# ctlab/metafast

Hardware: AMD Instinct MI355X
Metric: k-mers/s counted+graphed at k=31, 150 bp reads (higher is better)
Workload: dtype u64

## Files before the change

### metafast_amd/csrc/mf_skm.hip

```cpp
#include "mf_common.h"
#include "mf_count_dev.h"
#include <algorithm>
#include <memory>
#include <vector>
#include "mf_skm_scan.h"
#include "mf_skm_scatter.h"
#include "mf_skm_split.h"
#include "mf_skm_count.h"

template <typename KF> static int skm_set_lds(KF kern, size_t bytes) {
    MF_HIP(hipFuncSetAttribute(reinterpret_cast<const void *>(kern), hipFuncAttributeMaxDynamicSharedMemorySize, (int)bytes));
    return MF_OK;
}

#define SKM_PILOT_CH 8192
__global__ __launch_bounds__(256) void k_skm_pilot(const skm_rec *__restrict__ recs, const uint64_t *__restrict__ pstart, const uint32_t *__restrict__ plen,
                                                   const uint32_t *__restrict__ regions, int shift, uint32_t nsel, uint32_t *__restrict__ cnt,
                                                   uint32_t *__restrict__ occ, const uint64_t *__restrict__ ostart, uint32_t *__restrict__ cur,
                                                   skm_rec *__restrict__ out) {
    extern __shared__ uint32_t sh[];
    const uint32_t rg = blockIdx.y, d1 = regions[rg];
    const uint64_t start = pstart[d1];
    const uint32_t len = plen[d1];
    const uint32_t j0 = blockIdx.x * (uint32_t)SKM_PILOT_CH;
    if (j0 >= len) return;
    const uint32_t j1 = min(len, j0 + (uint32_t)SKM_PILOT_CH);
    const bool hist = ostart == nullptr;
    if (hist) { for (uint32_t i = threadIdx.x; i < 2u * nsel; i += blockDim.x) sh[i] = 0; __syncthreads(); }
    for (uint32_t j = j0 + threadIdx.x; j < j1; j += blockDim.x) {
        const skm_rec v = recs[start + j];
        if (!skm_rec_valid(v)) continue;
        const uint32_t d = skm_rec_digits(v) >> shift;
        if (d >= nsel) continue;
        if (hist) { atomicAdd(&sh[d], 1u); atomicAdd(&sh[nsel + d], skm_rec_n(v)); }
        else { const uint32_t at = atomicAdd(&cur[rg * nsel + d], 1u); out[ostart[rg * nsel + d] + at] = v; }
    }
    if (hist) {
        __syncthreads();
        for (uint32_t i = threadIdx.x; i < nsel; i += blockDim.x) {
            if (sh[i]) { atomicAdd(&cnt[rg * nsel + i], sh[i]); atomicAdd(&occ[rg * nsel + i], sh[nsel + i]); }
        }
    }
}
__global__ void k_skm_pilot_dir(const uint32_t *__restrict__ cnt, uint32_t n, uint32_t *__restrict__ plen) {
    const uint32_t i = blockIdx.x * blockDim.x + threadIdx.x;
    if (i < n) plen[i] = (cnt[i] + 3u) & ~3u;
}
template <int K>
static int skm_pilot(mf_ctx *ctx, const skm_rec *bufA, const uint64_t *pstart, const uint32_t *plen, uint32_t dlo, uint32_t dhi, uint64_t n_occ, int nd1,
                     int bits_planned, int kthr, double *rho, double *kept, double *rec_per_occ) {
    hipStream_t st = ctx->stream;
    *rho = -1.0; *kept = -1.0; *rec_per_occ = 0.0;
    if (dhi <= dlo) return MF_OK;
    const uint32_t R = std::min<uint32_t>(8u, dhi - dlo);
    const int pb = std::min((int)SKM_DIGIT_BITS, bits_planned + 3);
    const double per_unit = (double)n_occ / (double)nd1 / (double)(1u << pb);
    uint32_t nsel = (uint32_t)std::min<double>((double)(1u << pb), std::max(1.0, std::ceil(2.5e6 / (per_unit * R))));
    if (nsel > 2048u) nsel = 2048u;
    const uint32_t nb = R * nsel;
    std::vector<uint32_t> h_reg(R);
    for (uint32_t i = 0; i < R; i++) h_reg[i] = dlo + (uint32_t)(((uint64_t)(2 * i + 1) * (dhi - dlo)) / (2 * R));
    std::vector<uint32_t> h_len(nd1);
    mf_buf<uint32_t> reg, cnt, occ, cur, uplen, dcount; mf_buf<uint64_t> ostart, toff; mf_buf<unsigned long long> ps;
    MF_TRY(reg.alloc(ctx, R)); MF_TRY(cnt.alloc(ctx, (size_t)3 * nb)); MF_TRY(uplen.alloc(ctx, nb)); MF_TRY(dcount.alloc(ctx, nb));
    MF_TRY(ostart.alloc(ctx, (size_t)nb + 1)); MF_TRY(toff.alloc(ctx, (size_t)nb + 1)); MF_TRY(ps.alloc(ctx, 24));
    uint32_t *const d_cnt = cnt.p, *const d_occ = cnt.p + nb, *const d_cur = cnt.p + 2 * (size_t)nb;
    MF_HIP(hipMemcpyAsync(reg.p, h_reg.data(), (size_t)R * 4, hipMemcpyHostToDevice, st));
    MF_HIP(hipMemsetAsync(cnt.p, 0, (size_t)3 * nb * 4, st));
    MF_HIP(hipMemsetAsync(ps.p, 0, 24 * 8, st));
    const uint64_t mean_len = std::max<uint64_t>(1, n_occ / (uint64_t)nd1 / 4);
    const unsigned gx = (unsigned)std::min<uint64_t>(65535, (4 * mean_len + SKM_PILOT_CH - 1) / SKM_PILOT_CH + 1);
    const int shift = SKM_DIGIT_BITS - pb;
    mf_ktimer tm(ctx, "k_skm_pilot");
    k_skm_pilot<<<dim3(gx, R), 256, (size_t)2 * nsel * 4, st>>>(bufA, pstart, plen, reg.p, shift, nsel, d_cnt, d_occ, nullptr, nullptr, nullptr);
    k_skm_pilot_dir<<<(nb + 255) / 256, 256, 0, st>>>(d_cnt, nb, uplen.p);
    MF_TRY(mf_scan<1>(ctx, uplen.p, ostart.p, nb, (uint64_t *)&ps.p[0]));
    MF_TRY(mf_scan<1>(ctx, d_occ, toff.p, nb, (uint64_t *)&ps.p[1]));
    unsigned long long tot[2] = {0, 0};
    MF_HIP(hipMemcpyAsync(tot, ps.p, 16, hipMemcpyDeviceToHost, st));
    MF_HIP(hipStreamSynchronize(st));
    if (!tot[0] || !tot[1]) return MF_OK;
    mf_buf<skm_rec> pr; mf_buf<uint64_t> tkeys; mf_buf<uint16_t> tcnt;
    if (pr.alloc(ctx, tot[0] + 4) != MF_OK || tkeys.alloc(ctx, tot[1]) != MF_OK || tcnt.alloc(ctx, tot[1]) != MF_OK) return MF_OK;
    MF_HIP(hipMemsetAsync(pr.p, 0xFF, (tot[0] + 4) * sizeof(skm_rec), st));
    k_skm_pilot<<<dim3(gx, R), 256, 0, st>>>(bufA, pstart, plen, reg.p, shift, nsel, nullptr, nullptr, ostart.p, d_cur, pr.p);
    {
        const unsigned grid = (unsigned)std::min<uint64_t>(nb, (uint64_t)ctx->n_cu * C2_WG_PER_CU);
        k_skm_count<K><<<grid, SKM_CT, C2_LDS, st>>>(pr.p, ostart.p, uplen.p, nb, toff.p, tkeys.p, tcnt.p, dcount.p, (unsigned int *)&ps.p[2], 0u, (uint64_t)0, kthr,
                                                         &ps.p[3], (unsigned int *)&ps.p[4], nullptr, &ps.p[8], (uint64_t)tot[1], (uint32_t)ctx->opt_skm_dedupe, nullptr);
    }
    MF_TRY(mf_scan<1>(ctx, dcount.p, ostart.p, nb, (uint64_t *)&ps.p[5]));
    unsigned long long res[4] = {0, 0, 0, 0};
    MF_HIP(hipMemcpyAsync(res, &ps.p[2], 32, hipMemcpyDeviceToHost, st));
    MF_HIP(hipStreamSynchronize(st));
    MF_HIP(hipGetLastError());
    const bool over = (res[0] & 0xFFFFFFFFull) != 0;
    *rho = over ? 1.0 : (double)res[1] / (double)tot[1];
    if (!over) *kept = (double)res[3] / (double)tot[1];
    *rec_per_occ = (double)tot[0] / (double)tot[1];
    if (ctx->opt_verbose)
        fprintf(stderr, "[mf] skm pilot: %u would-be units of %u regions (2^%d per region): %llu records, %llu occurrences, %llu distinct k-mers = %.4f per occurrence (%llu kept), %llu unit(s) redone\n",
                nb, R, pb, tot[0], tot[1], res[1], *rho, res[3], res[2] & 0xFFFFFFFFull);
    return MF_OK;
}

struct skm_snap_slice {
    std::vector<uint64_t> rec;
    std::vector<uint64_t> pstart, l1_pstart; std::vector<uint32_t> plen, pocc, l1_plen;
    std::vector<int> lv;
    uint64_t cap = 0, wpb = 0, n_valid = 0; uint32_t dlo = 0, dhi = 0; int G = 0, one_pass = 0, repeated = 0, fast = 0;
};
struct mf_skm_snap { std::vector<skm_snap_slice> slices; };
#define MF_SKM_SNAPPED 3
struct skm_acc {
    mf_skm_snap *snap = nullptr;
    mf_buf<uint64_t> dk; mf_buf<uint16_t> dc; uint64_t dused = 0, dcap = 0;
    mf_buf<uint64_t> doff;
    mf_buf<unsigned long long> dhist, c2p;
    unsigned long long n_records = 0, cap_l1 = 0;
    uint32_t np_total = 0;
    int split_bits = 1;
    int table_bits = 0;
};
#define MF_SKM_NOMEM 2
struct skm_shared {
    uint32_t lo = 0, hi = 0;
    bool ready = false;
    mf_buf<skm_rec> buf; mf_buf<uint64_t> pstart; mf_buf<uint32_t> plen, pocc;
    std::vector<uint64_t> h_pstart;
    unsigned long long cap = 0;
    void clear() { buf.reset(); pstart.reset(); plen.reset(); pocc.reset(); h_pstart.clear(); ready = false; cap = 0; }
};
struct skm_reads { const uint8_t *bases; uint64_t n_bases; const uint32_t *vmask; uint64_t n_words; };
struct skm_job { skm_reads in; uint64_t n_occ; unsigned long long *scal; int kthr; };
struct skm_l1 { skm_reads in; uint64_t wpb; int bits1, G; uint32_t lo, hi; size_t fast_lds; };
struct skm_slice_state {
    std::vector<int> &lv; int total_bits;
    uint32_t dlo, dhi;
    skm_l1 l1;
    uint32_t np; mf_buf<uint64_t> pstart; mf_buf<uint32_t> plen, pocc;
    mf_buf<skm_rec> bufA; unsigned long long cap = 0;
    uint64_t rebase = 0;
    int snap_one_pass = 0, snap_repeated = 0;
};
#define SKM_STEP(call) do { const int rc__ = (call); if (rc__ != MF_OK) return rc__; } while (0)

static size_t skm_fast_lds(const mf_ctx *ctx, int nd1) {
    const size_t fast_lds = ((skm_stage_bytes(nd1) + 15) & ~(size_t)15) + (size_t)16 * SKM_FAST_WAVE_BYTES;
    return fast_lds > (size_t)160 * 1024 || ctx->opt_scatter_fast == 0 ? 0 : fast_lds;
}
template <int K, bool DYN>
static int skm_scatter(mf_ctx *ctx, const skm_l1 &L, const uint64_t *blockstart, skm_rec *out, const skm_dyn &Dy) {
    hipStream_t st = ctx->stream;
    mf_ktimer t(ctx, "k_skm_scatter");
    if (L.fast_lds) {
        MF_TRY(skm_set_lds(k_skm_scatter<K, DYN, true>, L.fast_lds));
        k_skm_scatter<K, DYN, true><<<L.G, 1024, L.fast_lds, st>>>(L.in.bases, L.in.n_bases, L.in.vmask, L.in.n_words, L.wpb, L.bits1, blockstart, L.G, out, Dy, L.lo, L.hi);
    } else {
        const size_t lds = skm_stage_bytes(1 << L.bits1);
        MF_TRY(skm_set_lds(k_skm_scatter<K, DYN, false>, lds));
        k_skm_scatter<K, DYN, false><<<L.G, 1024, lds, st>>>(L.in.bases, L.in.n_bases, L.in.vmask, L.in.n_words, L.wpb, L.bits1, blockstart, L.G, out, Dy, L.lo, L.hi);
    }
    return MF_OK;
}
static unsigned long long skm_final_cap(const std::vector<int> &lv, uint64_t n_occ, unsigned long long c1, bool headroom) {
    const int nd1 = 1 << lv[0];
    if (headroom) return c1 + n_occ / 128 + (unsigned long long)nd1 * SKM_LINE * (1ull << MF_MAX_DIGIT_BITS);
    if (lv.size() < 3) return c1;
    unsigned long long c = c1, p = (unsigned long long)nd1;
    for (size_t li = 1; li < lv.size(); li++) { c += p * SKM_LINE * (1ull << lv[li]); p <<= lv[li]; }
    return c;
}

template <int K>
static int skm_level1(mf_ctx *ctx, const skm_job &J, skm_slice_state &T, bool own, bool headroom) {
    hipStream_t st = ctx->stream;
    unsigned long long *const scal = J.scal;
    const skm_l1 &L = T.l1;
    const int bits1 = L.bits1, nd1 = 1 << bits1, G = L.G;
    const uint32_t np = T.np;
    const bool l1_only = T.lv.size() == 1;
    auto final_cap = [&](unsigned long long c1) { return skm_final_cap(T.lv, J.n_occ, c1, headroom); };
    unsigned long long &cap = T.cap;
    bool dyn = !l1_only && (ctx->opt_skm_dyn == 2 || (ctx->opt_skm_dyn == 1 && L.in.n_words >= (1ull << 24)));
    for (int attempt = dyn ? 0 : 1; attempt < 2; attempt++) {
        const bool D = attempt == 0;
        const int stride = D ? (ctx->opt_skm_dyn == 2 ? 3 : 16) : 1;
        mf_buf<uint32_t> blockhist; MF_TRY(blockhist.alloc(ctx, (size_t)nd1 * G));
        mf_buf<uint32_t> blockocc; if (l1_only) MF_TRY(blockocc.alloc(ctx, (size_t)nd1 * G));
        {
            mf_ktimer t(ctx, D ? "k_skm_hist_sample" : "k_skm_hist");
            k_skm_hist<K><<<G, 1024, (size_t)nd1 * 8, st>>>(L.in.bases, L.in.n_bases, L.in.vmask, L.in.n_words, L.wpb, bits1, blockhist.p, blockocc.p, G, stride, L.lo, L.hi);
        }
        MF_DBG(ctx, "k_skm_hist");
        if (D) {
            mf_buf<uint32_t> rsize; MF_TRY(rsize.alloc(ctx, np));
            mf_buf<uint64_t> rstart; MF_TRY(rstart.alloc(ctx, (size_t)np + 1));
            mf_buf<unsigned long long> gcur; MF_TRY(gcur.alloc(ctx, np));
            k_skm_region_sizes<<<(nd1 + 255) / 256, 256, 0, st>>>(blockhist.p, G, nd1, (uint32_t)stride, rsize.p, L.lo, L.hi);
            MF_TRY(mf_scan<1>(ctx, rsize.p, rstart.p, np, (uint64_t *)&scal[1]));
            MF_HIP(hipMemcpyAsync(gcur.p, rstart.p, (size_t)np * 8, hipMemcpyDeviceToDevice, st));
            MF_HIP(hipMemsetAsync(&scal[5], 0, 8, st));
            MF_HIP(hipMemcpyAsync(&cap, &scal[1], 8, hipMemcpyDeviceToHost, st));
            MF_HIP(hipStreamSynchronize(st));
            if (T.bufA.alloc(ctx, std::max<unsigned long long>(cap + (uint64_t)G * SKM_CH, own ? final_cap(cap) : 0ull)) != MF_OK) return MF_SKM_NOMEM;
            skm_dyn Dy; Dy.gcur = gcur.p; Dy.rend = rstart.p + 1; Dy.overflow = (unsigned int *)&scal[5]; Dy.dump = cap; Dy.save = nullptr;
            MF_TRY((skm_scatter<K, true>(ctx, L, nullptr, T.bufA.p, Dy)));
            MF_DBG(ctx, "k_skm_scatter");
            k_skm_dir_dyn<<<(nd1 + 255) / 256, 256, 0, st>>>(rstart.p, gcur.p, nd1, T.pstart.p, T.plen.p);
            unsigned long long ovf = 0;
            MF_HIP(hipMemcpyAsync(&ovf, &scal[5], 8, hipMemcpyDeviceToHost, st));
            MF_HIP(hipStreamSynchronize(st));
            if (!ovf) { T.snap_one_pass = 1; break; }
            T.snap_repeated = 1;
            if (ctx->opt_verbose) fprintf(stderr, "[mf] skm: a sampled digit region was too small, level 1 again with exact ranges\n");
            T.bufA.reset();
            continue;
        }
        mf_buf<uint64_t> blockstart; MF_TRY(blockstart.alloc(ctx, (size_t)nd1 * G + 1));
        MF_TRY(mf_scan<SKM_LINE>(ctx, blockhist.p, blockstart.p, (uint64_t)nd1 * G, (uint64_t *)&scal[1]));
        MF_HIP(hipMemcpyAsync(&cap, &scal[1], 8, hipMemcpyDeviceToHost, st));
        MF_HIP(hipStreamSynchronize(st));
        if (T.bufA.alloc(ctx, own ? final_cap(cap) : cap) != MF_OK) return MF_SKM_NOMEM;
        MF_TRY((skm_scatter<K, false>(ctx, L, blockstart.p, T.bufA.p, skm_dyn())));
        MF_DBG(ctx, "k_skm_scatter");
        k_skm_dir<<<(nd1 + 255) / 256, 256, 0, st>>>(blockstart.p, blockocc.p, G, nd1, T.pstart.p, T.plen.p, T.pocc.p);
    }
    return MF_OK;
}

template <int K>
static int skm_share_level1(mf_ctx *ctx, skm_slice_state &T, skm_shared *SH, uint64_t n_occ) {
    hipStream_t st = ctx->stream;
    const int nd1 = 1 << T.l1.bits1;
    if (!SH->ready) {
        SH->buf.swap(T.bufA); SH->pstart.swap(T.pstart); SH->plen.swap(T.plen); SH->pocc.swap(T.pocc);
        SH->cap = T.cap;
        SH->h_pstart.resize(nd1);
        MF_HIP(hipMemcpyAsync(SH->h_pstart.data(), SH->pstart.p, (size_t)nd1 * 8, hipMemcpyDeviceToHost, st));
        MF_HIP(hipStreamSynchronize(st));
        SH->ready = true;
        if (T.l1.lo == 0 && T.l1.hi == (uint32_t)nd1 && n_occ) { ctx->last_l1_per_occ = (double)SH->cap / (double)n_occ; ctx->last_l1_k = K; }
    }
    T.bufA.borrow(ctx, SH->buf.p, SH->buf.n);
    MF_TRY(T.pstart.alloc(ctx, T.np)); MF_TRY(T.plen.alloc(ctx, T.np)); MF_TRY(T.pocc.alloc(ctx, T.np));
    MF_HIP(hipMemcpyAsync(T.pstart.p, SH->pstart.p, (size_t)nd1 * 8, hipMemcpyDeviceToDevice, st));
    MF_HIP(hipMemcpyAsync(T.plen.p, SH->plen.p, (size_t)nd1 * 4, hipMemcpyDeviceToDevice, st));
    T.rebase = SH->h_pstart[T.dlo];
    T.cap = (T.dhi < (uint32_t)nd1 ? SH->h_pstart[T.dhi] : SH->cap) - T.rebase;
    return MF_OK;
}

template <int K>
static int skm_replan_from_pilot(mf_ctx *ctx, const skm_job &J, skm_slice_state &T, skm_acc &A, bool *split_from_pilot) {
    const uint64_t n_occ = J.n_occ;
    const int kthr = J.kthr, bits1 = T.l1.bits1, nd1 = 1 << bits1;
    std::vector<int> &lv = T.lv;
    int &total_bits = T.total_bits;
    double rho = -1.0, kept = -1.0, rpo = 0.0;
    MF_TRY(skm_pilot<K>(ctx, T.bufA.p, T.pstart.p, T.plen.p, T.dlo, T.dhi, n_occ, nd1, total_bits - bits1, kthr, &rho, &kept, &rpo));
    ctx->last_pilot_rho = rho; ctx->n_pilots++;
    if (rho > 0.0) {
        double want_units = (double)n_occ * rho / (double)std::max<int64_t>(64, ctx->opt_skm_unit_distinct);
        const int64_t unit_records = ctx->opt_skm_unit_records > 0 ? ctx->opt_skm_unit_records : (K >= 25 ? 2000 : 4000) * SKM_CT / 512;
        if (ctx->opt_skm_dedupe) want_units = std::max(want_units, (double)n_occ * rpo / (double)unit_records);
        int Bc = 0; while (Bc < 30 && (double)(1ull << Bc) < want_units) Bc++;
        const int r = std::max(1, std::min(Bc - bits1, std::min((int)SKM_DIGIT_BITS, 30 - bits1)));
        if (ctx->opt_verbose) fprintf(stderr, "[mf] skm pilot: %.4f distinct k-mers per occurrence -> %d bits after level 1 (planned from the occurrences alone: %d)\n", rho, r, total_bits - bits1);
        lv.resize(1);
        if (r <= MF_MAX_DIGIT_BITS) lv.push_back(r); else { lv.push_back((r + 1) / 2); lv.push_back(r / 2); }
        total_bits = 0; for (int b : lv) total_bits += b;
        if (kthr >= 0 && kept >= 0.0 && !A.doff.p) {
            const double per_unit = (double)n_occ * kept / (double)(1ull << total_bits);
            int sb = 0; while (sb < 4 && per_unit / (double)(1 << sb) > (double)ctx->opt_part_good) sb++;
            A.split_bits = sb; *split_from_pilot = true;
            if (ctx->opt_verbose) fprintf(stderr, "[mf] skm pilot: %.4f k-mers per occurrence survive the cut: %.0f per counting unit -> %d table partition(s) per unit\n", kept, per_unit, 1 << sb);
        }
    }
    return MF_OK;
}

static int skm_plan_table(mf_ctx *ctx, int total_bits, bool split_from_pilot, skm_acc &A) {
    if (!split_from_pilot) A.split_bits = A.table_bits > 0 ? std::max(0, std::min(4, A.table_bits - total_bits)) : 1;
    if (total_bits + A.split_bits > 30) A.split_bits = 30 - total_bits;
    A.np_total = (uint32_t)(1ull << (total_bits + A.split_bits));
    MF_TRY(A.doff.alloc(ctx, (size_t)A.np_total + 1));
    return MF_OK;
}

static int skm_restrict_to_slice(mf_ctx *ctx, skm_slice_state &T) {
    hipStream_t st = ctx->stream;
    const uint32_t dlo = T.dlo, np = T.dhi - T.dlo;
    T.np = np;
    mf_buf<uint64_t> ps; MF_TRY(ps.alloc(ctx, np)); mf_buf<uint32_t> pl, po; MF_TRY(pl.alloc(ctx, np)); MF_TRY(po.alloc(ctx, np));
    MF_HIP(hipMemcpyAsync(ps.p, T.pstart.p + dlo, (size_t)np * 8, hipMemcpyDeviceToDevice, st));
    MF_HIP(hipMemcpyAsync(pl.p, T.plen.p + dlo, (size_t)np * 4, hipMemcpyDeviceToDevice, st));
    MF_HIP(hipMemcpyAsync(po.p, T.pocc.p + dlo, (size_t)np * 4, hipMemcpyDeviceToDevice, st));
    T.pstart.swap(ps); T.plen.swap(pl); T.pocc.swap(po);
    return MF_OK;
}

static int skm_snapshot_level1(mf_ctx *ctx, const skm_slice_state &T, skm_snap_slice &snap) {
    hipStream_t st = ctx->stream;
    const uint32_t np = T.np;
    snap.l1_pstart.resize(np); snap.l1_plen.resize(np);
    MF_HIP(hipMemcpyAsync(snap.l1_pstart.data(), T.pstart.p, (size_t)np * 8, hipMemcpyDeviceToHost, st));
    MF_HIP(hipMemcpyAsync(snap.l1_plen.data(), T.plen.p, (size_t)np * 4, hipMemcpyDeviceToHost, st));
    MF_HIP(hipStreamSynchronize(st));
// ... 783 lines not shown
```

### metafast_amd/csrc/mf_skm_scan.h

```cpp
#pragma once
#include "mf_common.h"
#include "mf_count_dev.h"

typedef ulonglong2 skm_rec;
typedef uint32_t skm_v4 __attribute__((ext_vector_type(4)));
#define SKM_LINE 4
#define SKM_QCAP 16
#define SKM_DIGIT_BITS 22
#define SKM_CT 512
#define SKM_NW (SKM_CT / 64)

__device__ __forceinline__ bool skm_rec_valid(const skm_rec &r) { return ((uint32_t)r.y & 63u) != 63u; }
__device__ __forceinline__ uint32_t skm_rec_n(const skm_rec &r) { return (uint32_t)r.y & 63u; }
__device__ __forceinline__ uint32_t skm_rec_digits(const skm_rec &r) { return (uint32_t)(r.y >> 6) & ((1u << SKM_DIGIT_BITS) - 1u); }

template <int K> struct skm_word {
    static constexpr int W = K - mf_skm_m(K) + 1;
    static constexpr int NM = 31 + W;
    static constexpr int RMAX = (MF_SKM_BASES - (K - 1)) < 20 ? (MF_SKM_BASES - (K - 1)) : 20;
    uint32_t D[4];
    uint32_t mh[32];
    uint32_t valid;
    uint32_t cut;
};

template <int K>
__device__ __forceinline__ void skm_cut_mask(skm_word<K> &S, uint32_t m) {
    uint32_t acc = 0;
#pragma unroll
    for (int j = 31; j >= 1; j--)
        asm("v_cmp_eq_u32 vcc, %1, %2\n\tv_addc_co_u32 %0, vcc, %0, %0, vcc" : "+v"(acc) : "v"(S.mh[j]), "v"(S.mh[j - 1]) : "vcc");
    const uint32_t same = acc << 1;
    S.cut = m & ~(same & (m << 1));
}

__device__ __forceinline__ uint32_t skm_rc16(uint32_t d) {
    const uint32_t r = __brev(~d);
    return ((r & 0xAAAAAAAAu) >> 1) | ((r & 0x55555555u) << 1);
}
template <int M>
__device__ __forceinline__ uint32_t skm_mmer_at(const uint32_t (&X)[4], int p) {
    const int q = p >> 4, o = p & 15;
    const uint32_t top = o ? __builtin_amdgcn_alignbit(X[q], q + 1 < 4 ? X[q + 1] : 0u, 32 - 2 * o) : X[q];
    return top >> (32 - 2 * M);
}

template <int K>
__device__ __forceinline__ void skm_scan_tail(skm_word<K> &S, uint32_t (&hs)[skm_word<K>::NM], uint32_t m) {
    constexpr int W = skm_word<K>::W, NM = skm_word<K>::NM;
    static_assert(W >= 3 && W <= 18, "window");
    auto min3 = [](uint32_t a, uint32_t b, uint32_t c) { const uint32_t m = a < b ? a : b; return m < c ? m : c; };
#pragma unroll
    for (int i = 0; i + 2 < NM; i++) hs[i] = min3(hs[i], hs[i + 1], hs[i + 2]);
    if (W >= 9) {
#pragma unroll
        for (int i = 0; i + 8 < NM; i++) hs[i] = min3(hs[i], hs[i + 3], hs[i + 6]);
#pragma unroll
        for (int j = 0; j < 32; j++) S.mh[j] = hs[j] < hs[j + W - 9] ? hs[j] : hs[j + W - 9];
    } else {
        constexpr int D = W - 3 < 3 ? W - 3 : 3;
#pragma unroll
        for (int j = 0; j < 32; j++) S.mh[j] = min3(hs[j], hs[j + D], hs[j + W - 3]);
    }
    skm_cut_mask<K>(S, m);
}

template <int K>
__device__ __forceinline__ void skm_scan_word(skm_word<K> &S, const uint8_t *__restrict__ bases, uint64_t n_bases, uint64_t w, uint32_t m) {
    constexpr int NM = skm_word<K>::NM, M = mf_skm_m(K);
    const uint64_t b0 = w * 32;
    const uint4 *p = reinterpret_cast<const uint4 *>(bases + (b0 < n_bases ? b0 : 0));
    const bool in1 = b0 + 16 < n_bases, in2 = b0 + 32 < n_bases, in3 = b0 + 48 < n_bases;
    const uint4 c0 = p[0], c1 = p[in1 ? 1 : 0], c2 = p[in2 ? 2 : 0], c3 = p[in3 ? 3 : 0];
    S.D[0] = b0 < n_bases ? mf_dec16(c0) : 0u; S.D[1] = in1 ? mf_dec16(c1) : 0u; S.D[2] = in2 ? mf_dec16(c2) : 0u; S.D[3] = in3 ? mf_dec16(c3) : 0u;
    S.valid = m;
    uint32_t hs[NM];
    const uint32_t R[4] = {skm_rc16(S.D[3]), skm_rc16(S.D[2]), skm_rc16(S.D[1]), skm_rc16(S.D[0])};
#pragma unroll
    for (int i = 0; i < NM; i++) {
        const uint32_t f = skm_mmer_at<M>(S.D, i), r = skm_mmer_at<M>(R, 64 - M - i);
        hs[i] = mf_mmer_hash(f < r ? f : r, M);
    }
    skm_scan_tail<K>(S, hs, m);
}
__device__ __forceinline__ uint32_t skm_from_next_lane(uint32_t v) {
    return (uint32_t)__builtin_amdgcn_update_dpp(0, (int)v, 0x130 , 0xF, 0xF, false);
}
__device__ __forceinline__ uint32_t skm_from_prev_lane(uint32_t v) {
    return (uint32_t)__builtin_amdgcn_update_dpp(0, (int)v, 0x138 , 0xF, 0xF, false);
}
template <int K>
__device__ __forceinline__ void skm_scan_word_halo(skm_word<K> &S, const uint8_t *__restrict__ bases, uint64_t n_bases, uint64_t w, uint32_t m) {
    constexpr int NM = skm_word<K>::NM, M = mf_skm_m(K);
    const uint64_t b0 = w * 32;
    const uint4 *p = reinterpret_cast<const uint4 *>(bases + (b0 < n_bases ? b0 : 0));
    const bool in1 = b0 + 16 < n_bases;
    const uint4 c0 = p[0], c1 = p[in1 ? 1 : 0];
    S.D[0] = b0 < n_bases ? mf_dec16(c0) : 0u; S.D[1] = in1 ? mf_dec16(c1) : 0u;
    S.D[2] = skm_from_next_lane(S.D[0]); S.D[3] = skm_from_next_lane(S.D[1]);
    S.valid = m;
    static_assert(64 - M - 31 >= 16, "reversed words");
    const uint32_t R3 = skm_rc16(S.D[0]);
    const uint32_t R[4] = {0u, skm_from_next_lane(R3), skm_rc16(S.D[1]), R3};
    uint32_t hs[34];
#pragma unroll
    for (int i = 0; i < 32; i++) {
        const uint32_t f = skm_mmer_at<M>(S.D, i), r = skm_mmer_at<M>(R, 64 - M - i);
        hs[i] = mf_mmer_hash(f < r ? f : r, M);
    }
    constexpr int W = skm_word<K>::W;
    static_assert(W >= 3 && W <= 18, "window");
    static_assert(NM <= 64, "halo");
    auto min3 = [](uint32_t a, uint32_t b, uint32_t c) { const uint32_t m = a < b ? a : b; return m < c ? m : c; };
    hs[32] = skm_from_next_lane(hs[0]); hs[33] = skm_from_next_lane(hs[1]);
    uint32_t a[38];
#pragma unroll
    for (int i = 0; i < 32; i++) a[i] = min3(hs[i], hs[i + 1], hs[i + 2]);
    if (W >= 9) {
        uint32_t b[32 + 9];
#pragma unroll
        for (int i = 32; i < 38; i++) a[i] = skm_from_next_lane(a[i - 32]);
#pragma unroll
        for (int i = 0; i < 32; i++) b[i] = min3(a[i], a[i + 3], a[i + 6]);
#pragma unroll
        for (int i = 32; i < 32 + W - 9; i++) b[i] = skm_from_next_lane(b[i - 32]);
#pragma unroll
        for (int j = 0; j < 32; j++) S.mh[j] = b[j] < b[j + W - 9] ? b[j] : b[j + W - 9];
    } else {
        constexpr int D = W - 3 < 3 ? W - 3 : 3;
#pragma unroll
        for (int i = 32; i < 32 + W - 3; i++) a[i] = skm_from_next_lane(a[i - 32]);
#pragma unroll
        for (int j = 0; j < 32; j++) S.mh[j] = min3(a[j], a[j + D], a[j + W - 3]);
    }
    skm_cut_mask<K>(S, m);
}

__device__ __forceinline__ uint32_t skm_sel(uint32_t a, uint32_t b, unsigned long long m) {
    uint32_t r;
    asm("v_cndmask_b32 %0, %1, %2, %3" : "=v"(r) : "v"(a), "v"(b), "s"(m));
    return r;
}
template <int K>
__device__ __forceinline__ uint32_t skm_mh_at(const skm_word<K> &S, uint32_t s) {
    uint32_t a[16], b[8], c[4], d[2];
    const unsigned long long s0 = __ballot((s & 1u) != 0), s1 = __ballot((s & 2u) != 0), s2 = __ballot((s & 4u) != 0),
                             s3 = __ballot((s & 8u) != 0), s4 = __ballot((s & 16u) != 0);
#pragma unroll
    for (int i = 0; i < 16; i++) a[i] = skm_sel(S.mh[2 * i], S.mh[2 * i + 1], s0);
#pragma unroll
    for (int i = 0; i < 8; i++) b[i] = skm_sel(a[2 * i], a[2 * i + 1], s1);
#pragma unroll
    for (int i = 0; i < 4; i++) c[i] = skm_sel(b[2 * i], b[2 * i + 1], s2);
#pragma unroll
    for (int i = 0; i < 2; i++) d[i] = skm_sel(c[2 * i], c[2 * i + 1], s3);
    return skm_sel(d[0], d[1], s4);
}

template <int K>
__device__ __forceinline__ void skm_next_run(const skm_word<K> &S, uint32_t &cut, uint32_t &s, uint32_t &len) {
    s = (uint32_t)__builtin_ctz(cut);
    cut &= cut - 1u;
    const uint32_t stop = (cut | ~S.valid) & ~((2u << s) - 1u);
    const uint32_t e = stop ? (uint32_t)__builtin_ctz(stop) : 32u;
    len = e - s;
    if (len > (uint32_t)skm_word<K>::RMAX) { len = (uint32_t)skm_word<K>::RMAX; cut |= 1u << (s + len); }
}

template <int K>
__device__ __forceinline__ skm_rec skm_make_rec(const uint32_t (&D)[4], uint32_t s, uint32_t len, uint32_t digits, uint32_t D4 = 0u) {
    const uint32_t o = (2u * s) & 31u;
    const unsigned long long q = __ballot(s >= 16u);
    const uint32_t E0 = skm_sel(D[0], D[1], q), E1 = skm_sel(D[1], D[2], q), E2 = skm_sel(D[2], D[3], q), E3 = skm_sel(D[3], D4, q), E4 = skm_sel(D4, 0u, q);
    uint32_t T0 = E0, T1 = E1, T2 = E2, T3 = E3;
    if (o) {
        T0 = __builtin_amdgcn_alignbit(E0, E1, 32u - o);
        T1 = __builtin_amdgcn_alignbit(E1, E2, 32u - o);
        T2 = __builtin_amdgcn_alignbit(E2, E3, 32u - o);
        T3 = __builtin_amdgcn_alignbit(E3, E4, 32u - o);
    }
    static_assert(K >= 17 && K <= 32, "the first dword is kept whole");
    const int kb = 2 * (int)(len + K - 1);
    const uint64_t m01 = (uint64_t)((int64_t)0x8000000000000000ull >> ((kb < 64 ? kb : 64) - 1));
    const uint64_t m23 = ~(~0ull >> (kb > 64 ? kb - 64 : 0));
    T1 &= (uint32_t)m01; T2 &= (uint32_t)(m23 >> 32); T3 &= (uint32_t)m23;
    skm_rec r;
    r.x = ((uint64_t)T0 << 32) | T1;
    r.y = ((uint64_t)T2 << 32) | (uint64_t)(T3 & 0xF0000000u) | ((uint64_t)digits << 6) | (uint64_t)len;
    return r;
}
__device__ __forceinline__ void skm_route(uint32_t mh, int bits1, uint32_t &d1, uint32_t &digits) {
    const uint32_t ph = mf_remix32(mh);
    d1 = bits1 ? ph >> (32 - bits1) : 0u;
    digits = (bits1 ? (ph << bits1) : ph) >> (32 - SKM_DIGIT_BITS);
}
```

### metafast_amd/csrc/mf_skm_scatter.h

```cpp
#pragma once
#include "mf_skm_scan.h"

template <int K>
__global__ __launch_bounds__(1024) void k_skm_hist(const uint8_t *__restrict__ bases, uint64_t n_bases, const uint32_t *__restrict__ vmask,
                                                   uint64_t n_words, uint64_t words_per_block, int bits1,
                                                   uint32_t *__restrict__ blockhist, uint32_t *__restrict__ blockocc, int G, int stride,
                                                   uint32_t dlo, uint32_t dhi) {
    extern __shared__ __attribute__((aligned(16))) unsigned char smem[];
    const int nd = 1 << bits1;
    uint32_t *hist = reinterpret_cast<uint32_t *>(smem), *occ = hist + nd;
    for (int i = threadIdx.x; i < 2 * nd; i += blockDim.x) hist[i] = 0;
    __syncthreads();
    const uint64_t wlo = (uint64_t)blockIdx.x * words_per_block;
    const uint64_t whi = wlo + words_per_block < n_words ? wlo + words_per_block : n_words;
    for (uint64_t wb = wlo; wb < whi; wb += (uint64_t)blockDim.x * (uint64_t)stride) {
        const uint64_t w = wb + threadIdx.x;
        const uint32_t m = w < whi ? vmask[w] : 0u;
        if (__ballot(m != 0u) == 0ull) continue;
        skm_word<K> S;
        skm_scan_word<K>(S, bases, n_bases, w < n_words ? w : 0, m);
        uint32_t cut = S.cut;
        while (__ballot(cut != 0u) != 0ull) {
            if (cut) {
                uint32_t s, len, d1, digits;
// ... 40 lines not shown
                 "s_mov_b64 exec, %5\n\tds_read_b32 %0, %9\n\t"
                 "s_mov_b64 exec, %6\n\tds_read_b32 %1, %10\n\t"
                 "s_mov_b64 exec, %7\n\tds_read_b32 %2, %11\n\t"
                 "s_mov_b64 exec, %8\n\tds_read_b32 %3, %12\n\t"
                 "s_mov_b64 exec, %4\n\ts_waitcnt lgkmcnt(0)"
                 : "=&v"(v[0]), "=&v"(v[1]), "=&v"(v[2]), "=&v"(v[3]), "=&s"(sv)
                 : "s"(m[0]), "s"(m[1]), "s"(m[2]), "s"(m[3]), "v"(a[0]), "v"(a[1]), "v"(a[2]), "v"(a[3])
                 : "memory");
}
__device__ __forceinline__ void skm_lds_add_rtn4_if(const unsigned long long (&m)[4], const uint32_t (&a)[4], uint32_t inc, uint32_t (&old)[4]) {
    unsigned long long sv;
    asm volatile("s_mov_b64 %4, exec\n\t"
                 "s_mov_b64 exec, %5\n\tds_add_rtn_u32 %0, %9, %13\n\t"
                 "s_mov_b64 exec, %6\n\tds_add_rtn_u32 %1, %10, %13\n\t"
                 "s_mov_b64 exec, %7\n\tds_add_rtn_u32 %2, %11, %13\n\t"
                 "s_mov_b64 exec, %8\n\tds_add_rtn_u32 %3, %12, %13\n\t"
                 "s_mov_b64 exec, %4\n\ts_waitcnt lgkmcnt(0)"
                 : "=&v"(old[0]), "=&v"(old[1]), "=&v"(old[2]), "=&v"(old[3]), "=&s"(sv)
                 : "s"(m[0]), "s"(m[1]), "s"(m[2]), "s"(m[3]), "v"(a[0]), "v"(a[1]), "v"(a[2]), "v"(a[3]), "v"(inc)
                 : "memory");
}
__device__ __forceinline__ void skm_lds_write4_add_rtn4_if(const unsigned long long (&m)[4], const uint32_t (&wa)[4], const skm_v4 (&wv)[4],
                                                           const uint32_t (&a)[4], uint32_t inc, uint32_t (&old)[4]) {
    unsigned long long sv;
    asm volatile("s_mov_b64 %4, exec\n\t"
                 "s_mov_b64 exec, %5\n\tds_write_b128 %9, %13\n\tds_add_rtn_u32 %0, %17, %21\n\t"
                 "s_mov_b64 exec, %6\n\tds_write_b128 %10, %14\n\tds_add_rtn_u32 %1, %18, %21\n\t"
                 "s_mov_b64 exec, %7\n\tds_write_b128 %11, %15\n\tds_add_rtn_u32 %2, %19, %21\n\t"
                 "s_mov_b64 exec, %8\n\tds_write_b128 %12, %16\n\tds_add_rtn_u32 %3, %20, %21\n\t"
                 "s_mov_b64 exec, %4\n\ts_waitcnt lgkmcnt(0)"
                 : "=&v"(old[0]), "=&v"(old[1]), "=&v"(old[2]), "=&v"(old[3]), "=&s"(sv)
                 : "s"(m[0]), "s"(m[1]), "s"(m[2]), "s"(m[3]), "v"(wa[0]), "v"(wa[1]), "v"(wa[2]), "v"(wa[3]),
                   "v"(wv[0]), "v"(wv[1]), "v"(wv[2]), "v"(wv[3]), "v"(a[0]), "v"(a[1]), "v"(a[2]), "v"(a[3]), "v"(inc)
                 : "memory");
}
#define SKM_CH 256
#define SKM_NONE (~0ull)
struct skm_dyn {
    unsigned long long *gcur;
    const uint64_t *rend;
    unsigned int *overflow;
    uint64_t dump;
    unsigned long long *save;
};
template <bool DYN>
__device__ __forceinline__ uint64_t skm_take_line(const skm_stage &L, uint32_t dg, const skm_dyn &Dy) {
    uint64_t pos = L.cur[dg];
    if (DYN && (pos == SKM_NONE || (pos & (uint64_t)(SKM_CH - 1)) == 0ull)) {
        pos = atomicAdd(&Dy.gcur[dg], (unsigned long long)SKM_CH);
        if (pos + SKM_CH > Dy.rend[dg]) { atomicExch(Dy.overflow, 1u); pos = Dy.dump; }
    }
    L.cur[dg] = pos + SKM_LINE;
    return pos;
}
template <bool DYN = false>
__device__ __forceinline__ void skm_stage_insert(const skm_stage &L, skm_rec *__restrict__ out, const uint32_t (&d)[4],
                                                 const skm_rec (&rec)[4], bool (&pending)[4], const skm_dyn &Dy = skm_dyn()) {
    const uint32_t ctr0 = mf_lds_addr(L.ctr), line0 = mf_lds_addr(L.line);
    skm_v4 wv[4];
    uint32_t ca[4], la[4];
#pragma unroll
    for (int b = 0; b < 4; b++) {
        wv[b].x = (uint32_t)rec[b].x; wv[b].y = (uint32_t)(rec[b].x >> 32); wv[b].z = (uint32_t)rec[b].y; wv[b].w = (uint32_t)(rec[b].y >> 32);
        ca[b] = ctr0 + 4u * d[b];
        la[b] = line0 + 16u * SKM_LINE * d[b];
    }
    for (;;) {
        unsigned long long P[4], R[4], G[4];
#pragma unroll
        for (int b = 0; b < 4; b++) P[b] = __ballot(pending[b]);
        if ((P[0] | P[1] | P[2] | P[3]) == 0ull) break;
        uint32_t w[4], old[4], old2[4], wa[4];
        bool got[4];
        skm_lds_read4_if(P, ca, w);
#pragma unroll
        for (int b = 0; b < 4; b++) { got[b] = pending[b] && (w[b] & 0xFFFFu) < (uint32_t)SKM_LINE; R[b] = __ballot(got[b]); }
        skm_lds_add_rtn4_if(R, ca, 1u, old);
#pragma unroll
        for (int b = 0; b < 4; b++) {
            got[b] = got[b] && (old[b] & 0xFFFFu) < (uint32_t)SKM_LINE;
            wa[b] = la[b] + 16u * (old[b] & (uint32_t)(SKM_LINE - 1));
            G[b] = __ballot(got[b]);
        }
        skm_lds_write4_add_rtn4_if(G, wa, wv, ca, 0x10000u, old2);
        uint64_t *qpos = L.q_pos + (threadIdx.x >> 6) * SKM_QCAP;
        uint32_t *qd = L.q_d + (threadIdx.x >> 6) * SKM_QCAP;
        const uint64_t lt_mask = (1ull << mf_lane()) - 1ull;
        bool fl4[4], anyfl = false;
#pragma unroll
        for (int b = 0; b < 4; b++) {
            fl4[b] = got[b] && (old2[b] >> 16) == (uint32_t)(SKM_LINE - 1);
            anyfl |= fl4[b];
            if (got[b]) pending[b] = false;
        }
        if (__ballot(anyfl) == 0ull) continue;
#pragma unroll
        for (int b = 0; b < 4; b++) {
            const bool fl = fl4[b];
            const unsigned long long F = __ballot(fl);
            if (F == 0ull) continue;
            const uint32_t n = (uint32_t)__popcll(F), qi = (uint32_t)__popcll(F & lt_mask);
            uint64_t mypos = 0;
            if (fl) mypos = skm_take_line<DYN>(L, d[b], Dy);
            for (uint32_t e0 = 0; e0 < n; e0 += SKM_QCAP) {
                if (fl && qi >= e0 && qi < e0 + SKM_QCAP) { qpos[qi - e0] = mypos; qd[qi - e0] = d[b]; }
                asm volatile("s_waitcnt lgkmcnt(0)" ::: "memory");
                const uint32_t e = e0 + ((uint32_t)mf_lane() >> 2), c = (uint32_t)mf_lane() & 3u;
                if (e < n) {
                    const uint32_t dd = qd[e - e0];
                    const uint64_t pp = qpos[e - e0];
                    const skm_rec v = L.line[dd * SKM_LINE + c];
                    out[pp + c] = v;
                    asm volatile("" ::: "memory");
                    if (c == 0) __hip_atomic_store(&L.ctr[dd], 0u, __ATOMIC_RELEASE, MF_WG);
                }
                asm volatile("s_waitcnt lgkmcnt(0)" ::: "memory");
            }
        }
        asm volatile("" ::: "memory");
        __builtin_amdgcn_wave_barrier();
    }
}
template <bool DYN = false>
__device__ __forceinline__ void skm_stage_flush_all(const skm_stage &L, skm_rec *__restrict__ out, int nd, const skm_dyn &Dy = skm_dyn()) {
    const skm_rec SENT = make_ulonglong2(~0ull, ~0ull);
    for (int d = threadIdx.x; d < nd; d += blockDim.x) {
        const uint32_t c = L.ctr[d] >> 16;
        if (c) {
            const uint64_t pos = skm_take_line<DYN>(L, (uint32_t)d, Dy);
            for (uint32_t s = 0; s < (uint32_t)SKM_LINE; s++) {
                skm_rec v = L.line[d * SKM_LINE + s];
                if (s >= c) v = SENT;
                out[pos + s] = v;
            }
            L.ctr[d] = 0;
        }
        if (DYN) {
            uint64_t pos = L.cur[d];
            if (Dy.save) Dy.save[(size_t)blockIdx.x * nd + d] = pos;
            else if (pos != SKM_NONE) for (; (pos & (uint64_t)(SKM_CH - 1)) != 0ull; pos++) out[pos] = SENT;
        }
    }
}
__global__ void k_skm_close_chunks(const unsigned long long *__restrict__ save, uint64_t n, uint64_t cap, skm_rec *__restrict__ out) {
    const uint64_t i = (uint64_t)blockIdx.x * blockDim.x + threadIdx.x;
    if (i >= n) return;
    uint64_t pos = save[i];
    if (pos == SKM_NONE || pos >= cap) return;
    const skm_rec SENT = make_ulonglong2(~0ull, ~0ull);
    for (; (pos & (uint64_t)(SKM_CH - 1)) != 0ull; pos++) out[pos] = SENT;
}

#define SKM_LCAP 384
#define SKM_FAST_WAVE_BYTES (64 * 16 + 64 * 8 + SKM_LCAP * 8)
template <int J0>
__device__ __forceinline__ void skm_runlist8(uint32_t &c, uint32_t &at, uint32_t lane, uint32_t h0, uint32_t h1, uint32_t h2, uint32_t h3,
                                             uint32_t h4, uint32_t h5, uint32_t h6, uint32_t h7) {
    uint32_t t;
    unsigned long long sv, m0, m1, m2, m3, m4, m5, m6, m7;
#define SKM_RL_STEP(M, H, J) "s_mov_b64 exec, %[" M "]\n\tv_lshl_or_b32 %[t], %[lane], 5, %[" J "]\n\tds_write2_b32 %[at], %[" H "], %[t] offset1:1\n\tv_add_u32 %[at], 8, %[at]\n\t"
    asm volatile("v_add_co_u32 %[c], %[m0], %[c], %[c]\n\tv_add_co_u32 %[c], %[m1], %[c], %[c]\n\t"
                 "v_add_co_u32 %[c], %[m2], %[c], %[c]\n\tv_add_co_u32 %[c], %[m3], %[c], %[c]\n\t"
                 "v_add_co_u32 %[c], %[m4], %[c], %[c]\n\tv_add_co_u32 %[c], %[m5], %[c], %[c]\n\t"
                 "v_add_co_u32 %[c], %[m6], %[c], %[c]\n\tv_add_co_u32 %[c], %[m7], %[c], %[c]\n\t"
                 "s_mov_b64 %[sv], exec\n\t"
                 SKM_RL_STEP("m0", "h0", "j0") SKM_RL_STEP("m1", "h1", "j1") SKM_RL_STEP("m2", "h2", "j2") SKM_RL_STEP("m3", "h3", "j3")
                 SKM_RL_STEP("m4", "h4", "j4") SKM_RL_STEP("m5", "h5", "j5") SKM_RL_STEP("m6", "h6", "j6") SKM_RL_STEP("m7", "h7", "j7")
                 "s_mov_b64 exec, %[sv]"
                 : [c] "+v"(c), [at] "+v"(at), [t] "=&v"(t), [sv] "=&s"(sv), [m0] "=&s"(m0), [m1] "=&s"(m1), [m2] "=&s"(m2), [m3] "=&s"(m3),
                   [m4] "=&s"(m4), [m5] "=&s"(m5), [m6] "=&s"(m6), [m7] "=&s"(m7)
                 : [lane] "v"(lane), [h0] "v"(h0), [h1] "v"(h1), [h2] "v"(h2), [h3] "v"(h3), [h4] "v"(h4), [h5] "v"(h5), [h6] "v"(h6), [h7] "v"(h7),
                   [j0] "i"(J0), [j1] "i"(J0 + 1), [j2] "i"(J0 + 2), [j3] "i"(J0 + 3), [j4] "i"(J0 + 4), [j5] "i"(J0 + 5), [j6] "i"(J0 + 6), [j7] "i"(J0 + 7)
                 : "memory");
#undef SKM_RL_STEP
}
template <int K, bool DYN, bool FAST>
__global__ __launch_bounds__(1024) void k_skm_scatter(const uint8_t *__restrict__ bases, uint64_t n_bases, const uint32_t *__restrict__ vmask,
                                                      uint64_t n_words, uint64_t words_per_block, int bits1,
                                                      const uint64_t *__restrict__ blockstart, int G, skm_rec *__restrict__ out, skm_dyn Dy,
                                                      uint32_t dlo, uint32_t dhi) {
    extern __shared__ __attribute__((aligned(16))) unsigned char smem[];
    const int nd = 1 << bits1;
    skm_stage L = skm_stage_carve(smem, nd);
    if (DYN) Dy.dump += (uint64_t)blockIdx.x * SKM_CH;
    for (int i = threadIdx.x; i < nd; i += blockDim.x) {
        L.cur[i] = DYN ? (Dy.save ? (uint64_t)Dy.save[(size_t)blockIdx.x * nd + i] : SKM_NONE) : blockstart[(size_t)i * G + blockIdx.x];
        L.ctr[i] = 0;
    }
    __syncthreads();
    const uint32_t lane = (uint32_t)mf_lane();
    unsigned char *wbase = smem + ((skm_stage_bytes(nd) + 15) & ~(size_t)15) + (size_t)(threadIdx.x >> 6) * SKM_FAST_WAVE_BYTES;
    uint4 *pd = reinterpret_cast<uint4 *>(wbase);
    uint2 *pc = reinterpret_cast<uint2 *>(wbase + 64 * 16);
    uint2 *rl = reinterpret_cast<uint2 *>(wbase + 64 * 16 + 64 * 8);
    const uint64_t wlo = (uint64_t)blockIdx.x * words_per_block;
    const uint64_t whi = wlo + words_per_block < n_words ? wlo + words_per_block : n_words;
    const uint64_t wstep = (uint64_t)(uint32_t)__builtin_amdgcn_readfirstlane((int)(blockDim.x >> 6)) * 63u;
    const uint64_t wave0 = (uint64_t)(uint32_t)__builtin_amdgcn_readfirstlane((int)(threadIdx.x >> 6)) * 63u;
    for (uint64_t wb = wlo; wb < whi; wb += wstep) {
        uint32_t wlo32 = (uint32_t)__builtin_amdgcn_readfirstlane((int)(uint32_t)(wb + wave0));
        uint32_t whi32 = (uint32_t)__builtin_amdgcn_readfirstlane((int)(uint32_t)((wb + wave0) >> 32));
        asm("" : "+s"(wlo32), "+s"(whi32));
        const uint64_t w = (((uint64_t)whi32 << 32) | wlo32) + lane;
        const uint32_t m = (lane < 63u && w < whi) ? vmask[w] : 0u;
        if (__ballot(m != 0u) == 0ull) continue;
        skm_word<K> S;
        skm_scan_word_halo<K>(S, bases, n_bases, w < n_words ? w : 0, m);
        uint32_t cut = S.cut;
        bool fast = FAST;
        uint32_t NR = 0, roff = 0, cutf = cut, ext = 0;
        if (FAST) {
            constexpr int R = skm_word<K>::RMAX;
            static_assert(R >= 16 && R <= 20, "run-length check");
            const uint32_t z = ~(cut | ~S.valid);
            const uint32_t z2 = z & (z >> 1), z4 = z2 & (z2 >> 2), z8 = z4 & (z4 >> 4), z16 = z8 & (z8 >> 8);
            const uint32_t zr = R == 16 ? z16 : (R == 17 ? (z16 & (z >> 16)) : (R == 18 ? (z16 & (z2 >> 16)) : (R == 19 ? (z16 & (z2 >> 16) & (z >> 18)) : (z16 & (z4 >> 16)))));
            const uint32_t pcut = skm_from_prev_lane(cut), pvalid = skm_from_prev_lane(S.valid), pm31 = skm_from_prev_lane(S.mh[31]);
            const bool cont = (S.valid & 1u) && (pvalid >> 31) && S.mh[0] == pm31;
            const uint32_t hstop = (cut & ~1u) | ~S.valid;
            const uint32_t h = hstop ? (uint32_t)__builtin_ctz(hstop) : 32u;
            const uint32_t tail = pcut ? (uint32_t)__builtin_clz(pcut) + 1u : 32u;
            constexpr uint32_t XMAX = 49 - K < R ? (uint32_t)(49 - K) : (uint32_t)R;
            uint32_t allowed = tail < (uint32_t)R ? (uint32_t)R - tail : 0u;
            if (allowed > XMAX) allowed = XMAX;
            ext = (DYN && cont) ? (h < allowed ? h : allowed) : 0u;
            cutf = ext ? ((cut & ~1u) | (ext < h ? (1u << ext) : 0u)) : cut;
            roff = mf_wave_excl_scan((uint32_t)__popc(cutf), &NR);
            fast = __ballot(zr != 0u) == 0ull && NR <= (uint32_t)SKM_LCAP;
        }
        if (FAST && fast) {
            pd[lane] = make_uint4(S.D[0], S.D[1], S.D[2], S.D[3]);
            pc[lane] = make_uint2(cutf | ~S.valid, ext);
            {
                uint32_t at = mf_lds_addr(rl) + 8u * roff, c = __brev(cutf);
                skm_runlist8<0>(c, at, lane, S.mh[0], S.mh[1], S.mh[2], S.mh[3], S.mh[4], S.mh[5], S.mh[6], S.mh[7]);
                skm_runlist8<8>(c, at, lane, S.mh[8], S.mh[9], S.mh[10], S.mh[11], S.mh[12], S.mh[13], S.mh[14], S.mh[15]);
                skm_runlist8<16>(c, at, lane, S.mh[16], S.mh[17], S.mh[18], S.mh[19], S.mh[20], S.mh[21], S.mh[22], S.mh[23]);
                skm_runlist8<24>(c, at, lane, S.mh[24], S.mh[25], S.mh[26], S.mh[27], S.mh[28], S.mh[29], S.mh[30], S.mh[31]);
            }
            asm volatile("s_waitcnt lgkmcnt(0)" ::: "memory");
            __builtin_amdgcn_wave_barrier();
            for (uint32_t g0 = 0; g0 < NR; g0 += 256) {
                uint32_t d[4]; skm_rec rec[4]; bool pend[4];
#pragma unroll
                for (int b = 0; b < 4; b++) {
                    const uint32_t g = g0 + 64u * (uint32_t)b + lane;
                    pend[b] = g < NR;
                    const uint2 de = rl[pend[b] ? g : 0u];
                    const uint32_t src = (de.y >> 5) & 63u, s0 = de.y & 31u;
                    const uint4 Dw = pd[src]; const uint2 cv = pc[src];
                    const uint4 Dn = pd[(src + 1u) & 63u]; const uint2 cn = pc[(src + 1u) & 63u];
                    const uint32_t stop = cv.x & ~((2u << s0) - 1u);
                    const uint32_t e = stop ? (uint32_t)__builtin_ctz(stop) : 32u;
                    const uint32_t len = e - s0 + (e == 32u ? cn.y : 0u);
                    const uint32_t DD[4] = {Dw.x, Dw.y, Dw.z, Dw.w};
                    uint32_t digits;
                    skm_route(de.x, bits1, d[b], digits);
                    rec[b] = skm_make_rec<K>(DD, s0, len, digits, Dn.z);
                    if (d[b] < dlo || d[b] >= dhi) pend[b] = false;
                }
                skm_stage_insert<DYN>(L, out, d, rec, pend, Dy);
            }
            asm volatile("s_waitcnt lgkmcnt(0)" ::: "memory");
            __builtin_amdgcn_wave_barrier();
            continue;
        }
        while (__ballot(cut != 0u) != 0ull) {
            uint32_t d[4]; skm_rec rec[4]; bool pend[4];
#pragma unroll
            for (int b = 0; b < 4; b++) {
                pend[b] = cut != 0u;
                d[b] = 0; rec[b] = make_ulonglong2(~0ull, ~0ull);
                if (pend[b]) {
                    uint32_t s, len, digits;
                    skm_next_run<K>(S, cut, s, len);
                    skm_route(skm_mh_at<K>(S, s), bits1, d[b], digits);
                    rec[b] = skm_make_rec<K>(S.D, s, len, digits);
                    if (d[b] < dlo || d[b] >= dhi) { pend[b] = false; d[b] = 0; }
                }
            }
            skm_stage_insert<DYN>(L, out, d, rec, pend, Dy);
        }
    }
    __syncthreads();
    skm_stage_flush_all<DYN>(L, out, nd, Dy);
}

__global__ void k_skm_region_sizes(const uint32_t *__restrict__ blockhist, int G, int nd, uint32_t scale, uint32_t *__restrict__ rsize,
                                   uint32_t dlo, uint32_t dhi) {
    const int d = blockIdx.x * blockDim.x + threadIdx.x;
    if (d >= nd) return;
    if ((uint32_t)d < dlo || (uint32_t)d >= dhi) { rsize[d] = 0; return; }
    uint64_t t = 0;
    for (int b = 0; b < G; b++) t += blockhist[(size_t)d * G + b];
    t *= scale;
    t += t / 16 + (uint64_t)G * SKM_CH + 8192;
    t = (t + SKM_CH - 1) & ~(uint64_t)(SKM_CH - 1);
    rsize[d] = t > 0xFFFFFF00ull ? 0xFFFFFF00u : (uint32_t)t;
}
__global__ void k_skm_dir_dyn(const uint64_t *__restrict__ rstart, const unsigned long long *__restrict__ gcur, int nd,
                              uint64_t *__restrict__ pstart, uint32_t *__restrict__ plen) {
    const int d = blockIdx.x * blockDim.x + threadIdx.x;
    if (d >= nd) return;
    pstart[d] = rstart[d];
    plen[d] = (uint32_t)(gcur[d] - rstart[d]);
}

__global__ void k_skm_dir(const uint64_t *__restrict__ blockstart, const uint32_t *__restrict__ blockocc, int G, int nd,
                          uint64_t *__restrict__ pstart, uint32_t *__restrict__ plen, uint32_t *__restrict__ pocc) {
    const int d = blockIdx.x * blockDim.x + threadIdx.x;
    if (d >= nd) return;
    const uint64_t s = blockstart[(size_t)d * G], e = blockstart[(size_t)(d + 1) * G];
    pstart[d] = s;
    plen[d] = (uint32_t)(e - s);
    if (blockocc) {
        uint64_t t = 0;
        for (int b = 0; b < G; b++) t += blockocc[(size_t)d * G + b];
        pocc[d] = t > 0xFFFFFFFFull ? 0xFFFFFFFFu : (uint32_t)t;
    }
}
```

Before: 92.49 billion.

## Pack per-lane scatter state into one LDS record, specialize unsliced scatter, asm base decode

Merges the per-lane word and cut arrays in LDS into a single 16-byte record per lane, with a zero sentinel at index 64. The next lane's words now come from adjacent records instead of a separate wraparound lookup, which cuts LDS footprint and the number of LDS reads per run. Adds a SLICE=false kernel instantiation that skips the digit-range check when the whole range is covered. Also makes the run-loop bound wave-uniform so empty sub-batches are skipped, and replaces the base decoder with a hand-written bit-interleave asm sequence. The asm decoder has to produce exactly the same packing as mf_dec16, and the halo/neighbor semantics change for lane 63.

```diff
diff --git a/metafast_amd/csrc/mf_skm.hip b/metafast_amd/csrc/mf_skm.hip
--- a/metafast_amd/csrc/mf_skm.hip
+++ b/metafast_amd/csrc/mf_skm.hip
@@ -153,7 +153,10 @@
 static int skm_scatter(mf_ctx *ctx, const skm_l1 &L, const uint64_t *blockstart, skm_rec *out, const skm_dyn &Dy) {
     hipStream_t st = ctx->stream;
     mf_ktimer t(ctx, "k_skm_scatter");
-    if (L.fast_lds) {
+    if (L.fast_lds && L.lo == 0u && L.hi == (1u << L.bits1)) {
+        MF_TRY(skm_set_lds(k_skm_scatter<K, DYN, true, false>, L.fast_lds));
+        k_skm_scatter<K, DYN, true, false><<<L.G, 1024, L.fast_lds, st>>>(L.in.bases, L.in.n_bases, L.in.vmask, L.in.n_words, L.wpb, L.bits1, blockstart, L.G, out, Dy, L.lo, L.hi);
+    } else if (L.fast_lds) {
         MF_TRY(skm_set_lds(k_skm_scatter<K, DYN, true>, L.fast_lds));
         k_skm_scatter<K, DYN, true><<<L.G, 1024, L.fast_lds, st>>>(L.in.bases, L.in.n_bases, L.in.vmask, L.in.n_words, L.wpb, L.bits1, blockstart, L.G, out, Dy, L.lo, L.hi);
     } else {
diff --git a/metafast_amd/csrc/mf_skm_scan.h b/metafast_amd/csrc/mf_skm_scan.h
--- a/metafast_amd/csrc/mf_skm_scan.h
+++ b/metafast_amd/csrc/mf_skm_scan.h
@@ -34,6 +34,19 @@
     S.cut = m & ~(same & (m << 1));
 }
 
+__device__ __forceinline__ uint32_t skm_dec16(uint4 v) {
+    uint32_t r, p, q;
+    asm("v_lshrrev_b32 %0, 1, %3\n\tv_lshlrev_b32 %1, 1, %4\n\tv_bfi_b32 %0, %7, %1, %0\n\t"
+        "v_lshlrev_b32 %1, 3, %5\n\tv_bfi_b32 %0, %8, %1, %0\n\tv_lshlrev_b32 %1, 5, %6\n\tv_bfi_b32 %0, %9, %1, %0\n\t"
+        "v_lshlrev_b32 %1, 1, %0\n\tv_xor_b32 %1, %1, %0\n\tv_lshrrev_b32 %2, 1, %0\n\tv_bfi_b32 %0, %10, %1, %2\n\t"
+        "v_lshlrev_b32 %1, 20, %0\n\tv_lshrrev_b32 %2, 20, %0\n\tv_bfi_b32 %0, %11, %1, %0\n\tv_bfi_b32 %0, %12, %2, %0\n\t"
+        "v_lshlrev_b32 %1, 10, %0\n\tv_lshrrev_b32 %2, 10, %0\n\tv_bfi_b32 %0, %13, %1, %0\n\tv_bfi_b32 %0, %14, %2, %0"
+        : "=&v"(r), "=&v"(p), "=&v"(q)
+        : "v"(v.x), "v"(v.y), "v"(v.z), "v"(v.w), "s"(0x0C0C0C0Cu), "s"(0x30303030u), "s"(0xC0C0C0C0u), "s"(0xAAAAAAAAu),
+          "s"(0xF0F00000u), "s"(0x00000F0Fu), "s"(0xCC00CC00u), "s"(0x00330033u));
+    return r;
+}
+
 __device__ __forceinline__ uint32_t skm_rc16(uint32_t d) {
     const uint32_t r = __brev(~d);
     return ((r & 0xAAAAAAAAu) >> 1) | ((r & 0x55555555u) << 1);
@@ -72,7 +85,7 @@
     const uint4 *p = reinterpret_cast<const uint4 *>(bases + (b0 < n_bases ? b0 : 0));
     const bool in1 = b0 + 16 < n_bases, in2 = b0 + 32 < n_bases, in3 = b0 + 48 < n_bases;
     const uint4 c0 = p[0], c1 = p[in1 ? 1 : 0], c2 = p[in2 ? 2 : 0], c3 = p[in3 ? 3 : 0];
-    S.D[0] = b0 < n_bases ? mf_dec16(c0) : 0u; S.D[1] = in1 ? mf_dec16(c1) : 0u; S.D[2] = in2 ? mf_dec16(c2) : 0u; S.D[3] = in3 ? mf_dec16(c3) : 0u;
+    S.D[0] = b0 < n_bases ? skm_dec16(c0) : 0u; S.D[1] = in1 ? skm_dec16(c1) : 0u; S.D[2] = in2 ? skm_dec16(c2) : 0u; S.D[3] = in3 ? skm_dec16(c3) : 0u;
     S.valid = m;
     uint32_t hs[NM];
     const uint32_t R[4] = {skm_rc16(S.D[3]), skm_rc16(S.D[2]), skm_rc16(S.D[1]), skm_rc16(S.D[0])};
@@ -96,7 +109,7 @@
     const uint4 *p = reinterpret_cast<const uint4 *>(bases + (b0 < n_bases ? b0 : 0));
     const bool in1 = b0 + 16 < n_bases;
     const uint4 c0 = p[0], c1 = p[in1 ? 1 : 0];
-    S.D[0] = b0 < n_bases ? mf_dec16(c0) : 0u; S.D[1] = in1 ? mf_dec16(c1) : 0u;
+    S.D[0] = b0 < n_bases ? skm_dec16(c0) : 0u; S.D[1] = in1 ? skm_dec16(c1) : 0u;
     S.D[2] = skm_from_next_lane(S.D[0]); S.D[3] = skm_from_next_lane(S.D[1]);
     S.valid = m;
     static_assert(64 - M - 31 >= 16, "reversed words");
diff --git a/metafast_amd/csrc/mf_skm_scatter.h b/metafast_amd/csrc/mf_skm_scatter.h
--- a/metafast_amd/csrc/mf_skm_scatter.h
+++ b/metafast_amd/csrc/mf_skm_scatter.h
@@ -216,7 +216,7 @@
 }
 
 #define SKM_LCAP 384
-#define SKM_FAST_WAVE_BYTES (64 * 16 + 64 * 8 + SKM_LCAP * 8)
+#define SKM_FAST_WAVE_BYTES (65 * 16 + SKM_LCAP * 8)
 template <int J0>
 __device__ __forceinline__ void skm_runlist8(uint32_t &c, uint32_t &at, uint32_t lane, uint32_t h0, uint32_t h1, uint32_t h2, uint32_t h3,
                                              uint32_t h4, uint32_t h5, uint32_t h6, uint32_t h7) {
@@ -238,7 +238,7 @@
                  : "memory");
 #undef SKM_RL_STEP
 }
-template <int K, bool DYN, bool FAST>
+template <int K, bool DYN, bool FAST, bool SLICE = true>
 __global__ __launch_bounds__(1024) void k_skm_scatter(const uint8_t *__restrict__ bases, uint64_t n_bases, const uint32_t *__restrict__ vmask,
                                                       uint64_t n_words, uint64_t words_per_block, int bits1,
                                                       const uint64_t *__restrict__ blockstart, int G, skm_rec *__restrict__ out, skm_dyn Dy,
@@ -254,9 +254,9 @@
     __syncthreads();
     const uint32_t lane = (uint32_t)mf_lane();
     unsigned char *wbase = smem + ((skm_stage_bytes(nd) + 15) & ~(size_t)15) + (size_t)(threadIdx.x >> 6) * SKM_FAST_WAVE_BYTES;
-    uint4 *pd = reinterpret_cast<uint4 *>(wbase);
-    uint2 *pc = reinterpret_cast<uint2 *>(wbase + 64 * 16);
-    uint2 *rl = reinterpret_cast<uint2 *>(wbase + 64 * 16 + 64 * 8);
+    uint4 *pk = reinterpret_cast<uint4 *>(wbase);
+    uint2 *rl = reinterpret_cast<uint2 *>(wbase + 65 * 16);
+    if (FAST && lane == 0) pk[64] = make_uint4(0u, 0u, 0u, 0u);
     const uint64_t wlo = (uint64_t)blockIdx.x * words_per_block;
     const uint64_t whi = wlo + words_per_block < n_words ? wlo + words_per_block : n_words;
     const uint64_t wstep = (uint64_t)(uint32_t)__builtin_amdgcn_readfirstlane((int)(blockDim.x >> 6)) * 63u;
@@ -293,8 +293,7 @@
             fast = __ballot(zr != 0u) == 0ull && NR <= (uint32_t)SKM_LCAP;
         }
         if (FAST && fast) {
-            pd[lane] = make_uint4(S.D[0], S.D[1], S.D[2], S.D[3]);
-            pc[lane] = make_uint2(cutf | ~S.valid, ext);
+            pk[lane] = make_uint4(S.D[0], S.D[1], cutf | ~S.valid, ext);
             {
                 uint32_t at = mf_lds_addr(rl) + 8u * roff, c = __brev(cutf);
                 skm_runlist8<0>(c, at, lane, S.mh[0], S.mh[1], S.mh[2], S.mh[3], S.mh[4], S.mh[5], S.mh[6], S.mh[7]);
@@ -304,24 +303,26 @@
             }
             asm volatile("s_waitcnt lgkmcnt(0)" ::: "memory");
             __builtin_amdgcn_wave_barrier();
-            for (uint32_t g0 = 0; g0 < NR; g0 += 256) {
+            const uint32_t NRs = (uint32_t)__builtin_amdgcn_readfirstlane((int)NR);
+            for (uint32_t g0 = 0; g0 < NRs; g0 += 256) {
                 uint32_t d[4]; skm_rec rec[4]; bool pend[4];
 #pragma unroll
                 for (int b = 0; b < 4; b++) {
+                    if (g0 + 64u * (uint32_t)b >= NRs) { pend[b] = false; d[b] = 0; rec[b] = make_ulonglong2(0ull, 0ull); continue; }
                     const uint32_t g = g0 + 64u * (uint32_t)b + lane;
-                    pend[b] = g < NR;
+                    pend[b] = g < NRs;
                     const uint2 de = rl[pend[b] ? g : 0u];
                     const uint32_t src = (de.y >> 5) & 63u, s0 = de.y & 31u;
-                    const uint4 Dw = pd[src]; const uint2 cv = pc[src];
-                    const uint4 Dn = pd[(src + 1u) & 63u]; const uint2 cn = pc[(src + 1u) & 63u];
-                    const uint32_t stop = cv.x & ~((2u << s0) - 1u);
+                    const uint4 P0 = pk[src], P1 = pk[src + 1u];
+                    const uint32_t D4 = reinterpret_cast<const uint32_t *>(pk + src + 2u)[0];
+                    const uint32_t stop = P0.z & ~((2u << s0) - 1u);
                     const uint32_t e = stop ? (uint32_t)__builtin_ctz(stop) : 32u;
-                    const uint32_t len = e - s0 + (e == 32u ? cn.y : 0u);
-                    const uint32_t DD[4] = {Dw.x, Dw.y, Dw.z, Dw.w};
+                    const uint32_t len = e - s0 + (e == 32u ? P1.w : 0u);
+                    const uint32_t DD[4] = {P0.x, P0.y, P1.x, P1.y};
                     uint32_t digits;
                     skm_route(de.x, bits1, d[b], digits);
-                    rec[b] = skm_make_rec<K>(DD, s0, len, digits, Dn.z);
-                    if (d[b] < dlo || d[b] >= dhi) pend[b] = false;
+                    rec[b] = skm_make_rec<K>(DD, s0, len, digits, D4);
+                    if (SLICE && (d[b] < dlo || d[b] >= dhi)) pend[b] = false;
                 }
                 skm_stage_insert<DYN>(L, out, d, rec, pend, Dy);
             }
@@ -340,7 +341,7 @@
                     skm_next_run<K>(S, cut, s, len);
                     skm_route(skm_mh_at<K>(S, s), bits1, d[b], digits);
                     rec[b] = skm_make_rec<K>(S.D, s, len, digits);
-                    if (d[b] < dlo || d[b] >= dhi) { pend[b] = false; d[b] = 0; }
+                    if (SLICE && (d[b] < dlo || d[b] >= dhi)) { pend[b] = false; d[b] = 0; }
                 }
             }
             skm_stage_insert<DYN>(L, out, d, rec, pend, Dy);
```

Result: no change. 93.07 billion, median of 6 (+0.6%).
